# dropbox/lepton

Measured on AMD Instinct MI355X. Metric: encode+decode MB/s (JPEG bytes/sec), bit-exact round trip, higher is better.
Workload: dtype int16/u8 (integer coder, no floating point)

## Files before the change

### lepton_amd/csrc/lep_enc5.h

```cpp
#pragma once
#include "lep_v3.h"
#include "lep_enc5_plan.h"
#ifdef LEP5_DEBUG
#include <cstdio>
#endif

namespace lep5 {
using namespace lep3;

constexpr int kRows = 64, kClasses = 10;
constexpr int kPRows = 63 + 14;
constexpr int kStreams = 2 * kRows * kClasses;
WDEV int stream_id(int ci, int row, int k) { return (ci * kRows + row) * kClasses + k; }
constexpr int kCoefSlice = 12 * 11 + 10 + 1;
constexpr int kSignSlice = 48, kNzSlice = 6 * 32, kEdgeNzSlice = 8 * 12, kDcSlice = 17 * 11 + 10 + 1;
constexpr uint32_t kThreshWords = 2u * 256 * 8 * 128;

WDEV uint32_t coef_entry(uint32_t vlow, int nres, int len, int bsr, int k, int u) {
    return vlow | ((uint32_t)nres << 10) | ((uint32_t)len << 14) | ((uint32_t)bsr << 18) | ((uint32_t)k << 23) | ((uint32_t)u << 27);
}
WDEV int coef_units(int len, int nres) { return ((len < 11 ? len + 1 : 11) + nres + 3) >> 2; }
WDEV uint32_t thresh_entry(uint32_t tbits, int n, int pcls, int lt, int u) {
    return tbits | ((uint32_t)n << 10) | ((uint32_t)pcls << 14) | ((uint32_t)lt << 23) | ((uint32_t)u << 27);
}
// ... 241 lines not shown
}
WDEV void fold_edgenz_wave(const SegPlan5* plans, uint8_t* arena, int seg0, int nseg, int ci, int vertical, int eob, FoldShared* sh) {
    fold_init(sh, kEdgeNzSlice);
    LANES(l) {
        const int seg = seg0 + l;
        if (seg < nseg) {
            const SegPlan5& P = plans[seg];
            const uint32_t* ctab = reinterpret_cast<const uint32_t*>(arena + P.arena_off + P.cls_base);
            const int c = (vertical ? kClsEv : kClsEh) + ci * 8 + eob;
            const uint32_t n = P.status ? 0u : ctab[kNumCls + c];
            uint32_t* rec = reinterpret_cast<uint32_t*>(arena + P.arena_off + P.ens_base[vertical]) + (size_t)(n ? ctab[c] : 0u);
            FoldLane fl{sh->slice + fold_col(l)};
            U4 nxt = n ? ld4(rec) : U4{0, 0, 0, 0};
            for (uint32_t i = 0; i < n; i += 4) {
                U4 g = nxt;
                if (i + 4 < n) nxt = ld4(rec + i + 4);
                uint32_t w[4] = {g.x, g.y, g.z, g.w};
#pragma unroll
                for (int q = 0; q < 4; ++q) {
                    const int nzq = (int)w[q] & 7, ne = (int)(w[q] >> 3) & 7;
                    uint32_t probs = 0;
                    int so_far = 0;
#pragma unroll
                    for (int b = 2; b >= 0; --b) {
                        const uint32_t bit = (uint32_t)(ne >> b) & 1u;
                        probs |= fl.code(nzq * 12 + b * 4 + so_far, bit) << (8 * (2 - b));
                        so_far = (so_far << 1) | (int)bit;
                    }
                    w[q] = probs;
                }
                st4(rec + i, U4{w[0], w[1], w[2], w[3]});
            }
        }
    }
}
WDEV void fold_dc_wave(const SegPlan5* plans, uint8_t* arena, int seg0, int nseg, int a, FoldShared* sh) {
    fold_init(sh, kDcSlice);
    LANES(l) {
        const int seg = seg0 + l;
        if (seg < nseg) {
            const SegPlan5& P = plans[seg];
            const uint32_t* ctab = reinterpret_cast<const uint32_t*>(arena + P.arena_off + P.cls_base);
            const uint32_t n = P.status ? 0u : ctab[kNumCls + kClsDc + a];
            uint32_t* rec = reinterpret_cast<uint32_t*>(arena + P.arena_off + P.dcs_base) + 6 * (size_t)(n ? ctab[kClsDc + a] : 0u);
            FoldLane fl{sh->slice + fold_col(l)};
            uint32_t nxt = n ? rec[0] : 0u;
            for (uint32_t i = 0; i < n; ++i) {
                const uint32_t e0 = nxt;
                if (i + 1 < n) nxt = rec[6 * (i + 1)];
                const int nu = coef_units((int)(e0 >> 14) & 15, (int)(e0 >> 10) & 15);
                for (int u = 0; u < nu; ++u) rec[6 * i + u] = fold_coef_unit(fl, e0 | ((uint32_t)u << 27), 17 * 11);
            }
        }
    }
}

struct BoolEnc5 {
    uint64_t low;
    uint32_t q24;
    int count;
    uint64_t stage;
    int nst;
    uint8_t* out;
    uint32_t pos, cap;
    uint32_t floor_;
    uint32_t carry_out;
    WDEV void init(uint8_t* o, uint32_t c) { out = o; cap = c; pos = 0; low = 0; q24 = 254u << 24; count = -24; stage = 0; nst = 0; floor_ = 0; carry_out = 0; }
    WDEV void bin(uint32_t bit, uint32_t prob) {
#if LEP_ON_GPU
        const uint32_t s = __umulhi(q24, prob);
#else
        const uint32_t s = (uint32_t)(((uint64_t)q24 * prob) >> 32);
#endif
        const uint32_t q = q24 >> 24;
        const uint32_t n = bit ? q - s : s + 1;
        const int f = __builtin_clz(n);
        q24 = (n << f) - (1u << 24);
        low += bit ? s + 1 : 0u;
        low <<= f - 24;
        count += f - 24;
    }
    WDEV void ripple() {
        uint32_t x = pos;
        while (x > floor_ && (x > cap || out[x - 1] == 0xffu)) { if (x <= cap) out[x - 1] = 0; --x; }
        if (x > floor_) out[x - 1] = (uint8_t)(out[x - 1] + 1);
        else if (floor_) ++carry_out;
    }
    WDEV void flush() {
        const int nb = count >= 0 ? (count >> 3) + 1 : 0;
        count -= 8 * nb;
        const int keep = 32 + count;
        const uint64_t o = low >> keep;
        low &= (1ull << keep) - 1;
        stage = (stage << (8 * nb)) + o;
        nst += nb;
        if ((stage >> (8 * nst)) & 1u) { stage &= (1ull << (8 * nst)) - 1; ripple(); }
        if (nst >= 4) {
            const uint32_t v = (uint32_t)(stage >> (8 * (nst - 4)));
            if (pos + 4 <= cap) { const uint32_t be = __builtin_bswap32(v); __builtin_memcpy(out + pos, &be, 4); }
            else for (int i = 0; i < 4; ++i) if (pos + (uint32_t)i < cap) out[pos + i] = (uint8_t)(v >> (24 - 8 * i));
            pos += 4; nst -= 4;
            stage &= (1ull << (8 * nst)) - 1;
        }
    }
    WDEV uint32_t finish(bool* overflow) {
        flush();
// ... 1172 lines not shown
```

### lepton_amd/csrc/lep_gpu.hip

```cpp
#include <hip/hip_runtime.h>

#include <algorithm>
#include <cstdio>
#include <cstdlib>
#include <cstring>
#include <mutex>
#include <string>
#include <vector>

#include "../../include/lepton_mi355x.h"
#include "lep_buffers.h"

#define LEP_DEV __device__ __forceinline__
#include "lep_core.h"
#include "lep_enc3.h"
#include "lep_dec4.h"
#include "lep_enc5.h"
#include "lep_enc5_plan.h"
#include "lep_huff.h"
#include "lep_huffdec.h"
#include "lep_huffdec_simt.h"
#include "lep_huff_simt.h"
#include "lep_huffprog.h"
#include "lep_huffprog_simt.h"
// ... 180 lines not shown
        if (PHASE == 2) __builtin_amdgcn_s_setprio(3);
        if (PHASE == 0) lep5::wchunk_range_lane(plans[seg], bins, recs + (size_t)seg * K + k, k, K);
        else lep5::wchunk_code_lane(plans[seg], bins, segs[seg], streams, recs + (size_t)seg * K + k, k, K);
    } else {
        if (id >= nseg) return;
        if (PHASE == 1) { status[segs[id].slot] = 0; nbins_out[segs[id].slot] = plans[id].nbins; lep5::wchunk_link_lane(plans[id], bins, recs + (size_t)id * K, K); }
        else lep5::wchunk_stitch_lane(plans[id], segs[id], streams, stream_len, status, recs + (size_t)id * K, K);
    }
}
template <int PHASE>
__global__ __launch_bounds__(64) void lep_enc5_wchunk_part_kernel(const lep5::SegPlan5* __restrict__ plans, const uint16_t* __restrict__ bins, const SegDev* __restrict__ segs,
                                                              int nseg, int nparts, int c, int part, lep5::WChunk5* recs, uint8_t* streams, const uint8_t* __restrict__ arena,
                                                              int32_t* status, uint32_t* nbins_out) {
    __builtin_amdgcn_s_setprio(3);
    const int id = (int)(blockIdx.x * 64 + threadIdx.x);
    const int seg = PHASE == 1 ? id : id / c, s = PHASE == 1 ? 0 : id - seg * c;
    if (seg >= nseg) return;
    const lep5::SegPlan5& P = plans[seg];
    const lep5::Ckpt5* ck = reinterpret_cast<const lep5::Ckpt5*>(arena + P.arena_off + P.ckpt_base);
    lep5::WChunk5* r = recs + (size_t)seg * (size_t)(nparts * c);
    if (PHASE == 0) lep5::wchunk_range_cut(P, bins, r + part * c + s, lep5::part_chunk_cut(P, ck, part, s, nparts, c));
    else if (PHASE == 2) lep5::wchunk_code_cut(P, bins, segs[seg], streams, r + part * c + s, lep5::part_chunk_cut(P, ck, part, s, nparts, c));
    else {
        if (part == 0) status[segs[seg].slot] = 0;
        if (part + 1 == nparts) nbins_out[segs[seg].slot] = P.nbins;
        lep5::wchunk_link_cuts(P, bins, r, part * c, (part + 1) * c, [&](int j) { return lep5::part_chunk_cut(P, ck, j / c, j % c, nparts, c); });
    }
}
__global__ void lep_enc5_plan_kernel(const uint32_t* __restrict__ counts, lep5::SegPlan5* plans, int nseg) {
    const int s = (int)(blockIdx.x * blockDim.x + threadIdx.x);
    if (s < nseg) lep5::plan_segment(counts + (size_t)s * lep5::kCountWords, plans + s);
}
__global__ __launch_bounds__(64) void lep_enc5_offsets_kernel(lep5::SegPlan5* plans, int nseg, uint64_t* totals) {
    uint64_t a = 0, b = 0;
    for (int s0 = 0; s0 < nseg; s0 += 64) {
        const int s = s0 + (int)threadIdx.x;
        const uint32_t ab = s < nseg ? plans[s].arena_bytes : 0u, bc = s < nseg ? plans[s].bins_cap : 0u;
        int oa, ob;
        const int va = (int)(ab >> 8), vb = (int)(bc >> 7);
        const int ta = lepwave::wave_excl_scan(&va, &oa), tb = lepwave::wave_excl_scan(&vb, &ob);
        if (s < nseg) { plans[s].arena_off = a + ((uint64_t)(uint32_t)oa << 8); plans[s].bins_off = b + ((uint64_t)(uint32_t)ob << 7); }
        a += (uint64_t)(uint32_t)ta << 8; b += (uint64_t)(uint32_t)tb << 7;
    }
    if (threadIdx.x == 0) { totals[0] = a; totals[1] = b; }
}
__global__ void lep_enc5_fill_kernel(uint4* p, size_t n16, uint32_t v) {
    const uint4 x = make_uint4(v, v, v, v);
    for (size_t i = blockIdx.x * (size_t)blockDim.x + threadIdx.x; i < n16; i += (size_t)gridDim.x * blockDim.x) p[i] = x;
}
__global__ __launch_bounds__(64) void lep_enc5_bucket_kernel(const lep5::SegPlan5* __restrict__ plans, uint8_t* arena) {
    __shared__ lep5::BucketShared sh;
    lep5::bucket_wave(plans + blockIdx.x, arena, &sh);
}
struct Fold5CoefShared { uint16_t slice[lep5::kCoefSlice * 64]; };
__global__ __launch_bounds__(64) void lep_enc5_fold_coef_kernel(const lep5::SegPlan5* __restrict__ plans, uint8_t* arena, int nseg, int groups) {
    __shared__ Fold5CoefShared shc;
    const int grp = (int)blockIdx.x % groups, job = (int)blockIdx.x / groups;
    const int ci = job / 630, row = (job % 630) / 10, k = job % 10;
    const int sid = lep5::stream_id(ci, row, k), seg = grp * 64 + (int)threadIdx.x;
    const bool work = seg < nseg && !plans[seg].status && plans[seg].cnt[sid] != 0;
    if (!__ballot(work)) return;
    lep5::fold_coef_wave(plans, arena, grp * 64, nseg, sid, reinterpret_cast<lep5::FoldShared*>(&shc));
}
struct Fold5SmallShared { uint16_t slice[lep5::kEdgeNzSlice * 64]; };
__global__ __launch_bounds__(64) void lep_enc5_fold_small_kernel(const lep5::SegPlan5* __restrict__ plans, uint8_t* arena, uint32_t* thresh_models, int nseg, int groups, int job0) {
    __shared__ Fold5SmallShared shs;
    lep5::FoldShared* sh = reinterpret_cast<lep5::FoldShared*>(&shs);
    const int grp = (int)blockIdx.x % groups;
    int job = (int)blockIdx.x / groups + job0;
    const int seg0 = grp * 64;
    if (job < 2) { lep5::fold_sign_wave(plans, arena, seg0, nseg, job, sh); return; }
    job -= 2;
    if (job < 12) { const int ci = job / 6, lt = 2 + job % 6; lep5::fold_thresh_wave(plans, arena, thresh_models, seg0, nseg, lep5::stream_id(ci, 63, lt), ci, sh); return; }
    job -= 12;
    lep5::fold_edgenz_wave(plans, arena, seg0, nseg, job / 16, (job / 8) & 1, job & 7, sh);
}
constexpr int kFold5SmallJobs = 2 + 12 + 32;
__global__ __launch_bounds__(64) void lep_enc5_fold_big_kernel(const lep5::SegPlan5* __restrict__ plans, uint8_t* arena, int nseg, int groups, int job0) {
    __shared__ lep5::FoldShared sh;
    const int grp = (int)blockIdx.x % groups;
    int job = (int)blockIdx.x / groups + job0;
    const int seg0 = grp * 64;
    if (job < 12) { lep5::fold_dc_wave(plans, arena, seg0, nseg, job, &sh); return; }
    job -= 12;
    lep5::fold_nz_wave(plans, arena, seg0, nseg, job / 10, job % 10, &sh);
}
constexpr int kFold5BigJobs = 12 + 20;
__global__ __launch_bounds__(64) void lep_enc5_write_kernel(const lep5::SegPlan5* __restrict__ plans, const uint16_t* __restrict__ bins, const SegDev* __restrict__ segs,
                                                          int nseg, uint8_t* streams, uint32_t* stream_len, int32_t* status, uint32_t* nbins_out, uint8_t* arena,
                                                          int part, int nparts) {
    __builtin_amdgcn_s_setprio(3);
    const int seg0 = (int)blockIdx.x * 64, seg = seg0 + (int)threadIdx.x;
    if (seg < nseg) {
        if (part == 0) status[segs[seg].slot] = 0;
        if (part + 1 == nparts) nbins_out[segs[seg].slot] = plans[seg].nbins;
    }
    lep5::write_wave(plans, bins, segs, seg0, nseg, streams, stream_len, status, arena, part, nparts);
}

__global__ __launch_bounds__(64, 8) void lep_huffman_encode_kernel(const lephuff::HuffImage* __restrict__ images,
                                                                   const lephuff::HuffSegment* __restrict__ segs, uint8_t* out,
                                                                   uint32_t* out_len, lephuff::HuffEnd* ends) {
    __shared__ lephuff::HuffShared sh;
    const int s = blockIdx.x;
    const lephuff::HuffSegment seg = segs[s];
    if (seg.pad & lephuff::kHuffSegSimt) return;
    if (seg.pad & lephuff::kHuffSegRefuse) {
        if (threadIdx.x == 0) {
            out_len[s] = 0;
            if (ends) { lephuff::HuffEnd e; memset(&e, 0, sizeof e); e.pad = lephuff::kHuffEndRefused; ends[s] = e; }
        }
        return;
    }
    lephuff::HuffWave w;
    const uint32_t n = w.run(images + seg.image, seg, &sh, out);
    if (threadIdx.x == 0) out_len[s] = n;
    if (ends) w.export_end(ends + s);
}
__global__ __launch_bounds__(256) void lep_zero_kernel(uint4* p, size_t n16) {
    for (size_t i = (size_t)blockIdx.x * blockDim.x + threadIdx.x; i < n16; i += (size_t)gridDim.x * blockDim.x) p[i] = uint4{0u, 0u, 0u, 0u};
}
__global__ __launch_bounds__(leppack::kScanLanes) void lep_pack_offsets_kernel(const uint32_t* __restrict__ len, int n, uint64_t* __restrict__ dst_off) {
    leppack::offsets([len](int i) { return len[i]; }, n, dst_off);
}
__global__ __launch_bounds__(64) void lep_pack_copy_kernel(const uint8_t* __restrict__ src, const uint64_t* __restrict__ src_off, const uint32_t* __restrict__ len,
                                                           int n, uint8_t* __restrict__ dst, uint64_t dst_cap, const uint64_t* __restrict__ dst_off) {
    if (dst_off[n] > dst_cap) return;
    const int i = (int)blockIdx.x;
    leppack::copy_run(src + src_off[i], dst + dst_off[i], len[i], threadIdx.x & 63u);
}
__global__ __launch_bounds__(64 * lepsamples::kWavesPerGroup) void lep_samples_kernel(const lepsamples::PlaneRec* __restrict__ recs, const uint32_t* __restrict__ first, int nplanes) {
    __shared__ uint32_t tiles[lepsamples::kWavesPerGroup][lepsamples::kTileWords];
    const int wave = __builtin_amdgcn_readfirstlane((int)(threadIdx.x >> 6));
    const uint32_t unit = blockIdx.x * (uint32_t)lepsamples::kWavesPerGroup + (uint32_t)wave;
    if (unit >= first[nplanes]) return;
    lepsamples::wave_samples(recs, first, nplanes, unit, tiles[wave]);
}
__global__ __launch_bounds__(64 * lepsamples::kWavesPerGroup) void lep_samples_dc_kernel(const lepsamples::PlaneRec* __restrict__ recs, const uint32_t* __restrict__ first, int nplanes) {
    const int wave = __builtin_amdgcn_readfirstlane((int)(threadIdx.x >> 6));
    const uint32_t unit = blockIdx.x * (uint32_t)lepsamples::kWavesPerGroup + (uint32_t)wave;
// ... 128 lines not shown
    lephuff::prog_rst_reduce(scans + blockIdx.x, plans + blockIdx.x, outs, rows);
}
__global__ __launch_bounds__(64, 4) void lep_huffman_progressive_pipelined_kernel(const lephuff::ProgDecScan* __restrict__ scans, lephuff::HuffDecRow* rows,
                                                                                 const lephuff::ProgDeps* __restrict__ deps, uint32_t* progress, uint32_t* ticket) {
    __shared__ lephuff::HuffDecShared sh;
    uint32_t t = 0;
    if (threadIdx.x == 0) t = atomicAdd(ticket, 1u);
    const int k = __builtin_amdgcn_readfirstlane((int)t);
    lephuff::ProgDecWave w;
    w.run_scan<true>(scans + k, &sh, rows, deps + k, progress, k);
}

__global__ __launch_bounds__(64, 8) void lep_huffman_decode_kernel(const lephuff::HuffDecImage* __restrict__ images, lephuff::HuffDecRow* rows) {
    __shared__ lephuff::HuffDecShared sh;
    __builtin_amdgcn_s_setprio(3);
    lephuff::HuffDecWave w;
    w.run(images + blockIdx.x, &sh, rows);
}

__global__ __launch_bounds__(64) void lep_huffman_simt_settle_kernel(const lephuff::HuffDecImage* __restrict__ images, lephuff::SimtImage* si, const lephuff::SimtWave* waves,
                                                                     const lephuff::SimtSub* in, lephuff::SimtSub* out, int settle, lephuff::SimtSlots* slots) {
    __shared__ lephuff::SimtShared sh;
    extern __shared__ __attribute__((aligned(16))) unsigned char simt_columns[];
    const lephuff::SimtWave w = waves[blockIdx.x];
    lephuff::simt_guess_or_settle(images + w.image, &sh, si + w.image, in + si[w.image].first, out + si[w.image].first, w.first_sub, settle, slots,
                                  reinterpret_cast<lephuff::SimtColumns*>(simt_columns));
}
__global__ __launch_bounds__(64) void lep_huffman_simt_place_kernel(const lephuff::HuffDecImage* __restrict__ images, lephuff::SimtImage* si, const lephuff::SimtSub* sub,
                                                                    lephuff::SimtPlace* place, int passes, lephuff::HuffDecRow* rows, const lephuff::SimtSlots* slots) {
    const int i = (int)blockIdx.x;
    lephuff::simt_place(images + i, si + i, sub + si[i].first, place + si[i].first, passes, rows, slots);
}
__global__ __launch_bounds__(64) void lep_huffman_simt_write_kernel(const lephuff::HuffDecImage* __restrict__ images, lephuff::SimtImage* si, const lephuff::SimtWave* waves,
                                                                    const lephuff::SimtSub* sub, const lephuff::SimtPlace* place, lephuff::HuffDecRow* rows) {
    __shared__ lephuff::SimtShared sh;
    __shared__ lephuff::SimtTile tile;
    const lephuff::SimtWave w = waves[blockIdx.x];
    lephuff::simt_write(images + w.image, &sh, &tile, si + w.image, sub + si[w.image].first, place + si[w.image].first, rows, w.first_sub);
}
__global__ void lep_huffman_simt_finish_kernel(const lephuff::HuffDecImage* __restrict__ images, int nimg, lephuff::HuffDecRow* rows, const lephuff::SimtImage* si) {
    const int i = (int)(blockIdx.x * blockDim.x + threadIdx.x);
    if (i < nimg) lephuff::simt_finish(images + i, si + i, rows);
}

}

struct lep_gpu {
    int device = 0;
    hipStream_t stream = nullptr;
    hipEvent_t ev0 = nullptr, ev1 = nullptr;
    bool timed = false;
    bool released = false;
    lep5::Enc5Options opt;
    hipStream_t stream2 = nullptr, stream3 = nullptr;
    hipEvent_t ev_fork = nullptr, ev_join = nullptr, ev_join3 = nullptr;
    int huffprog_pipeline = 1;
    int huffprog_split = 0;
    int huffprogdec_rst = 1;
    uint32_t huffprogdec_rst_floor = lephuff::kRstPieceFloor;
    int huffprogdec_win = 1;
    int huffprog_simt = 1;
    int huffprog_simt_rst = 1;
    uint32_t huffprog_forms[4] = {0, 0, 0, 0};
    int cut_progressive = 0;
    int stream_pack = 1;
    int huffenc_simt = 1;
    int simt_sub_bits = 0;
    int huffprog_pipeline_max = 16384;
    hipEvent_t ev_part[8] = {nullptr, nullptr, nullptr, nullptr, nullptr, nullptr, nullptr, nullptr};
    int wchunks_parts = 0, wchunks_per_part = 0;
    std::vector<uint32_t> wchunks_slots;
    hipEvent_t ev_stage[8] = {nullptr, nullptr, nullptr, nullptr, nullptr, nullptr, nullptr, nullptr};
    int nstage = 0;
    int dec_company = 0;
    int dec_waves = 0;
    std::string err;
    const char* last_kernel = "";
    char simt_name[112] = "";
    struct Vmm {
        bool on = false;
        size_t chunk = (size_t)512 << 20;
        hipMemAllocationProp prop;
        hipMemAccessDesc access;
        std::vector<hipMemGenericAllocationHandle_t> pool;
        size_t mapped_total = 0, creates = 0, releases = 0;
    } vmm;
    enum Ws {
        W_ENC5_ENTRIES,
        W_ENC5_BINLIST,
        W_MODELS, W_MODELS_1,
        W_NS, W_NS_1,
        W_TRIMMED,
        W_META = W_TRIMMED, W_META_1,
        W_ROWS, W_ROWS_1,
        W_ENC5_PLANS,
        W_ENC5_WCHUNKS,
        W_BLOCKS, W_STREAMS, W_LENS,
        W_HUFF, W_HUFF_1,
        W_HUFFENC, W_HUFFENC_1,
        W_HUFFPROG, W_HUFFPROG_1,
        W_HUFFPROGSIMT, W_HUFFPROGSIMT_1,
        W_HUFFSEQ, W_HUFFSEQ_1,
        W_HUFFPROGDEC,
        W_HUFFPROGRST,
        W_HUFFDEC,
        W_HUFFPAR,
        W_PACK, W_PACK_1,
        W_SAMPLES, W_SAMPLES_1,
// ... 120 lines not shown
    }
    if (b.mapped > old) HIPCHK(g, hipMemSetAccess(b.va + old, b.mapped - old, &V.access, 1));
    w.set(b.va, b.mapped);
    return 0;
}
static int ensure(lep_gpu* g, Workspace& w, size_t need, bool may_release = true) {
    if (w.cap >= need) return 0;
    if (g->vmm.on && (need >= ((size_t)32 << 20) || w.v.va)) {
        if (!w.v.va) HIPCHK(g, w.release());
        return vmm_ensure(g, w, need, may_release);
    }
    hipError_t e = w.ensure(need, need / 8);
    if (e != hipSuccess && may_release) {
        (void)hipGetLastError();
        release_idle_caches(g);
        e = w.ensure(need);
    }
    if (e != hipSuccess) { g->err = std::string("hipMalloc: ") + hipGetErrorString(e); return LEP_GPU_ERROR; }
    return 0;
}

#include "lep_derive.h"


template <class Ready>
static int launch_enc5_writer(const lep5::Enc5WriterPlan& W, const lep5::SegPlan5* plans, const uint16_t* binlist, const SegDev* segs, int nseg, lep5::WChunk5* recs,
                              uint8_t* arena, uint8_t* streams, uint32_t* stream_len, int32_t* status, uint32_t* bins, hipStream_t wst, Ready&& ready) {
#define LEP_WCHUNK(PHASE, GRID) hipLaunchKernelGGL((lep_enc5_wchunk_kernel<PHASE>), dim3(GRID), dim3(64), 0, wst, plans, binlist, segs, nseg, W.records, recs, streams, stream_len, status, bins)
#define LEP_WPART(PHASE, GRID) hipLaunchKernelGGL((lep_enc5_wchunk_part_kernel<PHASE>), dim3(GRID), dim3(64), 0, wst, plans, binlist, segs, nseg, \
                                                  W.gather_parts, W.chunks, part, recs, streams, (const uint8_t*)arena, status, bins)
    for (int part = 0; part < W.gather_parts; ++part) {
        if (int rc = ready(part)) return rc;
        if (W.form == LEP_DEBUG_WRITE_LANE)
            hipLaunchKernelGGL(lep_enc5_write_kernel, dim3(W.groups), dim3(64), 0, wst, plans, binlist, segs, nseg, streams, stream_len, status, bins, arena, part, W.gather_parts);
        if (W.form == LEP_DEBUG_WRITE_PART_CHUNKS) { LEP_WPART(0, W.lane_groups); LEP_WPART(1, W.groups); LEP_WPART(2, W.lane_groups); }
    }
    if (int rc = ready(W.gather_parts)) return rc;
    if (W.form == LEP_DEBUG_WRITE_STITCHED) { LEP_WCHUNK(0, W.lane_groups); LEP_WCHUNK(1, W.groups); LEP_WCHUNK(2, W.lane_groups); }
    if (W.form != LEP_DEBUG_WRITE_LANE) LEP_WCHUNK(3, W.groups);
#undef LEP_WPART
#undef LEP_WCHUNK
    return 0;
}

constexpr int kEnc5NoMemory = -1000;
static int launch_enc5(lep_gpu* g, const ImageDev* d_img, const SegDev* d_seg, const uint64_t* d_nsoff, int nseg, uint8_t* d_streams,
                       uint32_t* d_stream_len, int32_t* d_status, hipStream_t st) {
    Workspace &models = g->ws[lep_gpu::W_MODELS + g->cur], &ns = g->ws[lep_gpu::W_NS + g->cur];
    Workspace &ws_plans = g->ws[lep_gpu::W_ENC5_PLANS], &ws_entries = g->ws[lep_gpu::W_ENC5_ENTRIES], &ws_binlist = g->ws[lep_gpu::W_ENC5_BINLIST], &wchunks = g->ws[lep_gpu::W_ENC5_WCHUNKS];
    if (!g->stream2) {
        HIPCHK(g, hipEventCreateWithFlags(&g->ev_enc5_done, hipEventDisableTiming));
        for (auto& e : g->ev_part) HIPCHK(g, hipEventCreateWithFlags(&e, hipEventDisableTiming));
        HIPCHK(g, hipStreamCreateWithFlags(&g->stream2, hipStreamNonBlocking));
        HIPCHK(g, hipStreamCreateWithFlags(&g->stream3, hipStreamNonBlocking));
        HIPCHK(g, hipEventCreateWithFlags(&g->ev_fork, hipEventDisableTiming));
        HIPCHK(g, hipEventCreateWithFlags(&g->ev_join, hipEventDisableTiming));
        HIPCHK(g, hipEventCreateWithFlags(&g->ev_join3, hipEventDisableTiming));
        for (auto& e : g->ev_stage) HIPCHK(g, hipEventCreate(&e));
    }
    lepbuf::Layout L;
    L.add<lep5::SegPlan5>((size_t)nseg);
    const size_t o_counts = L.add<uint32_t>((size_t)nseg * lep5::kCountWords), o_tot = L.add<uint64_t>(2);
    HIPCHK(g, hipStreamWaitEvent(st, g->ev_enc5_done, 0));
    if (int rc = ensure(g, ws_plans, L.padded())) return rc;
    lep5::SegPlan5* plans = ws_plans.at<lep5::SegPlan5>(0);
    uint32_t* counts = ws_plans.at<uint32_t>(o_counts);
    uint64_t* d_tot = ws_plans.at<uint64_t>(o_tot);
    const int groups = (nseg + 63) / 64;
    g->nstage = 0;
    HIPCHK(g, hipEventRecord(g->ev_stage[0], st));
    const bool two = g->opt.enc5_waves == 2;
    lep5::Enc5WriterPlan W = lep5::enc5_writer_plan(nseg, g->opt);
    int nparts = lep5::enc5_lane_plan(nseg, g->opt).gather_parts;
    auto walk =[&](int mode, uint8_t* entries, uint16_t* binlist, int part = 0) {
        size_t lds = lep5::walk_lds_bytes(mode);
        if (mode == lep5::kGather && g->opt.enc5_gather_wgs > 0) lds = std::max(lds, (size_t)(160 * 1024 / g->opt.enc5_gather_wgs) & ~(size_t)255);
#define LEP_WALK(MODE, NW) hipLaunchKernelGGL((lep_enc5_walk_kernel<MODE, NW>), dim3(nseg), dim3(64 * NW), lds, st, d_img, d_seg, (NSum*)ns.p, d_nsoff, plans, entries, binlist, counts, part, nparts)
        if (mode == lep5::kCount) { if (two) LEP_WALK(lep5::kCount, 2); else LEP_WALK(lep5::kCount, 1); }
        else if (mode == lep5::kEmit) { if (two) LEP_WALK(lep5::kEmit, 2); else LEP_WALK(lep5::kEmit, 1); }
        else { if (two) LEP_WALK(lep5::kGather, 2); else LEP_WALK(lep5::kGather, 1); }
#undef LEP_WALK
    };
    walk(lep5::kCount, nullptr, nullptr);
    hipLaunchKernelGGL(lep_enc5_plan_kernel, dim3(groups), dim3(64), 0, st, (const uint32_t*)counts, plans, nseg);
    hipLaunchKernelGGL(lep_enc5_offsets_kernel, dim3(1), dim3(64), 0, st, plans, nseg, d_tot);
    hipLaunchKernelGGL(lep_enc5_fill_kernel, dim3(4096), dim3(256), 0, st, (uint4*)models.p, (size_t)nseg * lep5::kThreshWords / 4, kBranchInit);
    uint64_t tot[2] = {0, 0};
    HIPCHK(g, hipMemcpyAsync(tot, d_tot, sizeof tot, hipMemcpyDeviceToHost, st));
    HIPCHK(g, hipStreamSynchronize(st));
    if ((size_t)tot[0] + (size_t)tot[1] * 2 > g->opt.enc5_scratch_max || ensure(g, ws_entries, (size_t)tot[0] + 256, false) || ensure(g, ws_binlist, (size_t)tot[1] * 2 + 256, false)) {
        (void)hipGetLastError();
        g->err.clear();
        static bool told = false;
        if (!told) { told = true; fprintf(stderr, "lepton-mi355x: no room for the split-phase encoder's scratch (%.1f GB for %d segments): single-kernel encoder\n", ((double)tot[0] + 2.0 * (double)tot[1]) / 1e9, nseg); }
        return kEnc5NoMemory;
    }
    if (W.records && ensure(g, wchunks, (size_t)nseg * W.records * sizeof(lep5::WChunk5) + 256, false)) { (void)hipGetLastError(); g->err.clear(); W = lep5::enc5_lane_plan(nseg, g->opt); }
    nparts = W.gather_parts;
    {
        HIPCHK(g, hipEventRecord(g->ev_stage[1], st));
        walk(lep5::kEmit, (uint8_t*)ws_entries.p, nullptr);
        HIPCHK(g, hipEventRecord(g->ev_stage[2], st));
        hipLaunchKernelGGL(lep_enc5_bucket_kernel, dim3(nseg), dim3(64), 0, st, (const lep5::SegPlan5*)plans, (uint8_t*)ws_entries.p);
        HIPCHK(g, hipEventRecord(g->ev_fork, st));
        HIPCHK(g, hipStreamWaitEvent(g->stream2, g->ev_fork, 0));
        HIPCHK(g, hipStreamWaitEvent(g->stream3, g->ev_fork, 0));
        if (g->opt.enc5_fold_apart) {
            const int small0[4] = {0, 2, 14, 46}, big0[3] = {0, 12, 32};
            for (int i = 0; i < 3; ++i)
                hipLaunchKernelGGL(lep_enc5_fold_small_kernel, dim3((unsigned)groups * (small0[i + 1] - small0[i])), dim3(64), 0, st, (const lep5::SegPlan5*)plans, (uint8_t*)ws_entries.p,
                                   (uint32_t*)models.p, nseg, groups, small0[i]);
            for (int i = 0; i < 2; ++i)
                hipLaunchKernelGGL(lep_enc5_fold_big_kernel, dim3((unsigned)groups * (big0[i + 1] - big0[i])), dim3(64), 0, st, (const lep5::SegPlan5*)plans, (uint8_t*)ws_entries.p, nseg, groups, big0[i]);
        } else {
        hipLaunchKernelGGL(lep_enc5_fold_small_kernel, dim3((unsigned)groups * kFold5SmallJobs), dim3(64), 0, g->stream2, (const lep5::SegPlan5*)plans, (uint8_t*)ws_entries.p,
                           (uint32_t*)models.p, nseg, groups, 0);
        hipLaunchKernelGGL(lep_enc5_fold_big_kernel, dim3((unsigned)groups * kFold5BigJobs), dim3(64), 0, g->stream3, (const lep5::SegPlan5*)plans, (uint8_t*)ws_entries.p, nseg, groups, 0);
        }
        hipLaunchKernelGGL(lep_enc5_fold_coef_kernel, dim3((unsigned)groups * 1260u), dim3(64), 0, st, (const lep5::SegPlan5*)plans, (uint8_t*)ws_entries.p, nseg, groups);
        HIPCHK(g, hipEventRecord(g->ev_join, g->stream2));
        HIPCHK(g, hipEventRecord(g->ev_join3, g->stream3));
        HIPCHK(g, hipStreamWaitEvent(st, g->ev_join, 0));
        HIPCHK(g, hipStreamWaitEvent(st, g->ev_join3, 0));
        HIPCHK(g, hipEventRecord(g->ev_stage[3], st));
        const hipStream_t wst = W.form == LEP_DEBUG_WRITE_STITCHED ? st : g->stream2;
        auto gathered = [&](int part) -> int {
            if (part == nparts) { HIPCHK(g, hipEventRecord(g->ev_stage[4], st)); return 0; }
            walk(lep5::kGather, (uint8_t*)ws_entries.p, (uint16_t*)ws_binlist.p, part);
            if (wst != st) { HIPCHK(g, hipEventRecord(g->ev_part[part], st)); HIPCHK(g, hipStreamWaitEvent(wst, g->ev_part[part], 0)); }
            return 0;
        };
        if (int rc = launch_enc5_writer(W, plans, (const uint16_t*)ws_binlist.p, d_seg, nseg, (lep5::WChunk5*)wchunks.p, (uint8_t*)ws_entries.p, d_streams, d_stream_len, d_status,
                                        g->d_bins, wst, gathered)) return rc;
        if (wst != st) { HIPCHK(g, hipEventRecord(g->ev_join, wst)); HIPCHK(g, hipStreamWaitEvent(st, g->ev_join, 0)); }
        HIPCHK(g, hipEventRecord(g->ev_stage[5], st));
        g->nstage = 5;
    }
    HIPCHK(g, hipEventRecord(g->ev_enc5_done, st));
    HIPCHK(g, hipGetLastError());
    g->wchunks_parts = W.report_parts; g->wchunks_per_part = W.chunks; g->last_kernel = W.name;
    return 0;
}

#define LEP_STAGED(T, N) static_assert(sizeof(T) == N, "a staged descriptor changed size: tests/test_stage_block.py WORKSPACES and tests/emu/stage_block_probe.cc ELEM_SIZES name it")
LEP_STAGED(ImageDev, 2208); LEP_STAGED(SegDev, 32); LEP_STAGED(lep_huff_image, 4272); LEP_STAGED(lep_huff_segment, 40); LEP_STAGED(lephuff::SimtEncSeg, 40);
LEP_STAGED(lephuff::SimtEncWave, 8); LEP_STAGED(lepsamples::PlaneRec, 176); LEP_STAGED(leprgb::RgbRec, 112); LEP_STAGED(lep_huffprog_image, 168); LEP_STAGED(lep_huffprog_scan, 4184);
LEP_STAGED(lephuff::ProgSimtScan, 48); LEP_STAGED(lephuff::ProgSimtWave, 8); LEP_STAGED(lephuff::ProgSimtRegion, 24); LEP_STAGED(lep_huffprogdec_scan, 5696);
LEP_STAGED(lephuff::ProgDeps, 16); LEP_STAGED(lephuff::ProgRstScan, 16); LEP_STAGED(lephuff::ProgRstOut, 24); LEP_STAGED(lep_huffdec_image, 5552);
LEP_STAGED(lephuff::SimtImage, 36); LEP_STAGED(lephuff::SimtWave, 8); LEP_STAGED(lephuff::SimtSub, 20); LEP_STAGED(lephuff::SimtPlace, 12); LEP_STAGED(lephuff::SimtSlots, 32);

static int stage(lep_gpu* g, Workspace& ws, const lepbuf::Block& B, hipStream_t st) {
    if (int rc = ensure(g, ws, B.padded())) return rc;
    const size_t n = B.upload_bytes();
    if (!n) return 0;
    lep_gpu::Staging& sl = g->staging[g->staging_next];
    g->staging_next = (g->staging_next + 1) % 16;
    if (sl.used) { HIPCHK(g, hipEventSynchronize(sl.ev)); sl.used = false; }
    if (!sl.ev) HIPCHK(g, hipEventCreateWithFlags(&sl.ev, hipEventDisableTiming));
    if (sl.cap < n) {
        if (sl.host) g->staging_retired.push_back(sl.host);
        sl.host = nullptr; sl.cap = 0;
        const size_t want = std::max<size_t>(n + n / 4 + 4096, (size_t)8 << 20);
        HIPCHK(g, hipHostMalloc(&sl.host, want, hipHostMallocDefault));
        sl.cap = want;
    }
    B.pack((char*)sl.host);
    HIPCHK(g, hipMemcpyAsync(ws.p, sl.host, n, hipMemcpyHostToDevice, st));
    HIPCHK(g, hipEventRecord(sl.ev, st));
    sl.used = true;
    return 0;
}

static int refuse_if_session(lep_gpu* g, const char* what) {
    if (!g->rows[g->cur].open) return 0;
    g->err = std::string(what) + ": arena set " + std::to_string(g->cur) + " belongs to a decode session until lep_gpu_decode_rows_end";
    return LEP_ASSERTION_FAILURE;
// ... 123 lines not shown
__attribute__((constructor)) static void lep_runtime_defaults() { setenv("GPU_MAX_HW_QUEUES", "8", 0); }

extern "C" {

static std::mutex g_live_mu;
static std::vector<lep_gpu*> g_live;
static bool g_exit_hook = false;
static void release_device_side(lep_gpu* g);
static void release_all_at_exit() {
    std::lock_guard<std::mutex> lk(g_live_mu);
    for (lep_gpu* g : g_live) release_device_side(g);
    g_live.clear();
}

int lep_gpu_create(int device, lep_gpu** out) {
    lep_gpu* g = new lep_gpu;
    g->device = device;
    if (const char* e = getenv("LEP_DEC_WAVES")) g->dec_waves = atoi(e) == 4 ? 4 : (atoi(e) == 8 ? 8 : 0);
    lep5::enc5_options_from_env(&g->opt);
    if (const char* e = getenv("LEP_HUFFPROG_PIPELINE")) g->huffprog_pipeline = atoi(e);
    if (const char* e = getenv("LEP_HUFFPROG_PIPELINE_MAX")) g->huffprog_pipeline_max = atoi(e);
    if (const char* e = getenv("LEP_HUFFDEC_SIMT_BITS")) g->simt_sub_bits = std::max(0, atoi(e));
    if (const char* e = getenv("LEP_HUFFENC_SIMT")) g->huffenc_simt = atoi(e) != 0;
    if (const char* e = getenv("LEP_STREAM_PACK")) g->stream_pack = atoi(e) != 0;
    if (const char* e = getenv("LEP_CUT_PROGRESSIVE")) g->cut_progressive = atoi(e) != 0;
    if (const char* e = getenv("LEP_HUFFPROG_SIMT")) g->huffprog_simt = atoi(e) != 0;
    if (const char* e = getenv("LEP_HUFFPROG_SIMT_RST")) g->huffprog_simt_rst = atoi(e) != 0;
    if (const char* e = getenv("LEP_HUFFPROGDEC_WIN")) g->huffprogdec_win = atoi(e) != 0;
    if (const char* e = getenv("LEP_HUFFPROGDEC_RST")) g->huffprogdec_rst = atoi(e) != 0;
    if (const char* e = getenv("LEP_HUFFPROGDEC_RST_FLOOR")) g->huffprogdec_rst_floor = (uint32_t)std::max(1, atoi(e));
    if (const char* e = getenv("LEP_HUFFPROG_SPLIT")) g->huffprog_split = atoi(e) != 0;
    int n = 0;
    if (hipGetDeviceCount(&n) != hipSuccess || n <= device) { delete g; return LEP_GPU_ERROR; }
    if (hipSetDevice(device) != hipSuccess || hipStreamCreate(&g->stream) != hipSuccess ||
        hipEventCreate(&g->ev0) != hipSuccess || hipEventCreate(&g->ev1) != hipSuccess) { delete g; return LEP_GPU_ERROR; }
    vmm_init(g);
    {
        std::lock_guard<std::mutex> lk(g_live_mu);
        g_live.push_back(g);
        if (!g_exit_hook) { g_exit_hook = true; atexit(release_all_at_exit); }
    }
    *out = g;
    return 0;
}

static void release_device_side(lep_gpu* g) {
    if (g->released) return;
    g->released = true;
    (void)hipSetDevice(g->device);
    (void)hipStreamSynchronize(g->stream);
    if (g->ev_enc5_done) (void)hipEventDestroy(g->ev_enc5_done);
    for (auto& e : g->ev_part) if (e) (void)hipEventDestroy(e);
    for (auto& e : g->ev_stage) if (e) (void)hipEventDestroy(e);
    if (g->ev_fork) (void)hipEventDestroy(g->ev_fork);
    if (g->ev_join) (void)hipEventDestroy(g->ev_join);
    if (g->ev_join3) (void)hipEventDestroy(g->ev_join3);
    if (g->stream2) (void)hipStreamDestroy(g->stream2);
    if (g->stream3) (void)hipStreamDestroy(g->stream3);
    for (Workspace& w : g->ws) dev_release(g, w);
    vmm_destroy(g);
    if (g->ev0) (void)hipEventDestroy(g->ev0);
    if (g->ev1) (void)hipEventDestroy(g->ev1);
    if (g->stream) (void)hipStreamDestroy(g->stream);
    for (lep_gpu::Staging& sl : g->staging) { if (sl.host) (void)hipHostFree(sl.host); if (sl.ev) (void)hipEventDestroy(sl.ev); sl = lep_gpu::Staging(); }
    for (void* p : g->staging_retired) (void)hipHostFree(p);
    g->staging_retired.clear();
}

void lep_gpu_destroy(lep_gpu* g) {
    if (!g) return;
    {
        std::lock_guard<std::mutex> lk(g_live_mu);
        for (size_t i = 0; i < g_live.size(); ++i) if (g_live[i] == g) { g_live.erase(g_live.begin() + i); break; }
        release_device_side(g);
    }
    delete g;
}

const char* lep_gpu_last_error(lep_gpu* g) { return g ? g->err.c_str() : "no gpu object"; }

int lep_gpu_encode_device(lep_gpu* g, const lep_image_desc* images, int nimg, const lep_segment* segs, int nseg,
                          uint8_t* d_streams, const uint64_t* stream_offsets, uint32_t* d_stream_len, int32_t* d_status,
                          void* hip_stream) {
    return launch<false>(g, images, nimg, segs, nseg, d_streams, stream_offsets, d_stream_len, d_status,
                         hip_stream ? (hipStream_t)hip_stream : g->stream);
}

int lep_gpu_decode_device(lep_gpu* g, const lep_image_desc* images, int nimg, const lep_segment* segs, int nseg,
                          const uint8_t* d_streams, const uint64_t* stream_offsets, const uint32_t* d_stream_len,
                          int32_t* d_status, void* hip_stream) {
    return launch<true>(g, images, nimg, segs, nseg, const_cast<uint8_t*>(d_streams), stream_offsets,
                        const_cast<uint32_t*>(d_stream_len), d_status, hip_stream ? (hipStream_t)hip_stream : g->stream);
}

int lep_gpu_decode_rows_begin(lep_gpu* g, const lep_image_desc* images, int nimg, const lep_segment* segs, int nseg,
                              const uint8_t* d_streams, const uint64_t* stream_offsets, const uint32_t* d_stream_len, void* hip_stream) {
    if (!g) return LEP_GPU_ERROR;
    if (int rc = refuse_if_session(g, "lep_gpu_decode_rows_begin")) return rc;
    if (nseg <= 0 || nimg <= 0) { g->err = "lep_gpu_decode_rows_begin: nothing to decode"; return LEP_ASSERTION_FAILURE; }
    hipStream_t st = hip_stream ? (hipStream_t)hip_stream : g->stream;
    LaunchFront F;
    if (int rc = launch_front(g, true, images, nimg, segs, nseg, stream_offsets, st, &F)) return rc;
    Workspace& recs = g->ws[lep_gpu::W_ROWS + g->cur];
    lepbuf::Layout L;
    L.add<lep4::Dec4Resume>((size_t)nseg);
    L.add<uint32_t>((size_t)nseg * kRowsLdsWords);
    if (int rc = ensure(g, recs, L.bytes())) return rc;
    HIPCHK(g, hipMemsetAsync(recs.p, 0, L.bytes(), st));
    lep_gpu::RowsSession& R = g->rows[g->cur];
    R.nseg = nseg; R.st = st; R.waves = decoder_waves(g, nseg);
    R.d_img = F.d_img; R.d_seg = F.d_seg; R.d_nsoff = F.d_nsoff; R.d_models = F.d_models; R.d_ns = F.d_ns;
// ... 835 lines not shown
```

Before: 1735.

## Merge three fold kernels into one launch and drop the extra streams

Replaces the separate small, big and coef fold kernels, which ran on three streams with fork/join events, with a single fold kernel that decodes a flat job index into a fold kind and dispatches to it. By default every fold job goes out in one grid on the main stream, removing the cross-stream events and two extra launches. All blocks now reserve the largest shared-memory layout, which can reduce occupancy for the small jobs. It also adds optional compile-time priority boosts for the sign and DC jobs, which are off by default.

```diff
diff --git a/lepton_amd/csrc/lep_enc5.h b/lepton_amd/csrc/lep_enc5.h
--- a/lepton_amd/csrc/lep_enc5.h
+++ b/lepton_amd/csrc/lep_enc5.h
@@ -317,6 +317,37 @@
                 for (int u = 0; u < nu; ++u) rec[6 * i + u] = fold_coef_unit(fl, e0 | ((uint32_t)u << 27), 17 * 11);
             }
         }
+    }
+}
+
+enum FoldKind { kFoldSign = 0, kFoldThresh, kFoldDc, kFoldNz, kFoldEdgeNz, kFoldCoef, kFoldKinds };
+constexpr int kFoldJobs = 2 + 12 + 12 + 20 + 32 + 1260;
+constexpr int fold_kind_job0(int kind) {
+    return kind <= kFoldSign ? 0 : kind == kFoldThresh ? 2 : kind == kFoldDc ? 14 : kind == kFoldNz ? 26 : kind == kFoldEdgeNz ? 46 : kind == kFoldCoef ? 78 : kFoldJobs;
+}
+struct FoldJob { int kind, a, b, c; };
+WDEV FoldJob fold_job(int job) {
+    if (job < 2) return FoldJob{kFoldSign, job, 0, 0};
+    job -= 2;
+    if (job < 12) return FoldJob{kFoldThresh, job / 6, 2 + job % 6, 0};
+    job -= 12;
+    if (job < 12) return FoldJob{kFoldDc, job, 0, 0};
+    job -= 12;
+    if (job < 20) return FoldJob{kFoldNz, job / 10, job % 10, 0};
+    job -= 20;
+    if (job < 32) return FoldJob{kFoldEdgeNz, job / 16, (job / 8) & 1, job & 7};
+    job -= 32;
+    return FoldJob{kFoldCoef, job / 630, (job % 630) / 10, job % 10};
+}
+WDEV void fold_run_job(int job, const SegPlan5* plans, uint8_t* arena, uint32_t* thresh_models, int seg0, int nseg, FoldShared* sh) {
+    const FoldJob j = fold_job(job);
+    switch (j.kind) {
+    case kFoldSign: fold_sign_wave(plans, arena, seg0, nseg, j.a, sh); break;
+    case kFoldThresh: fold_thresh_wave(plans, arena, thresh_models, seg0, nseg, stream_id(j.a, 63, j.b), j.a, sh); break;
+    case kFoldDc: fold_dc_wave(plans, arena, seg0, nseg, j.a, sh); break;
+    case kFoldNz: fold_nz_wave(plans, arena, seg0, nseg, j.a, j.b, sh); break;
+    case kFoldEdgeNz: fold_edgenz_wave(plans, arena, seg0, nseg, j.a, j.b, j.c, sh); break;
+    default: fold_coef_wave(plans, arena, seg0, nseg, stream_id(j.a, j.b, j.c), sh); break;
     }
 }
 
diff --git a/lepton_amd/csrc/lep_gpu.hip b/lepton_amd/csrc/lep_gpu.hip
--- a/lepton_amd/csrc/lep_gpu.hip
+++ b/lepton_amd/csrc/lep_gpu.hip
@@ -256,40 +256,27 @@
     __shared__ lep5::BucketShared sh;
     lep5::bucket_wave(plans + blockIdx.x, arena, &sh);
 }
-struct Fold5CoefShared { uint16_t slice[lep5::kCoefSlice * 64]; };
-__global__ __launch_bounds__(64) void lep_enc5_fold_coef_kernel(const lep5::SegPlan5* __restrict__ plans, uint8_t* arena, int nseg, int groups) {
-    __shared__ Fold5CoefShared shc;
-    const int grp = (int)blockIdx.x % groups, job = (int)blockIdx.x / groups;
-    const int ci = job / 630, row = (job % 630) / 10, k = job % 10;
-    const int sid = lep5::stream_id(ci, row, k), seg = grp * 64 + (int)threadIdx.x;
-    const bool work = seg < nseg && !plans[seg].status && plans[seg].cnt[sid] != 0;
-    if (!__ballot(work)) return;
-    lep5::fold_coef_wave(plans, arena, grp * 64, nseg, sid, reinterpret_cast<lep5::FoldShared*>(&shc));
-}
-struct Fold5SmallShared { uint16_t slice[lep5::kEdgeNzSlice * 64]; };
-__global__ __launch_bounds__(64) void lep_enc5_fold_small_kernel(const lep5::SegPlan5* __restrict__ plans, uint8_t* arena, uint32_t* thresh_models, int nseg, int groups, int job0) {
-    __shared__ Fold5SmallShared shs;
-    lep5::FoldShared* sh = reinterpret_cast<lep5::FoldShared*>(&shs);
-    const int grp = (int)blockIdx.x % groups;
-    int job = (int)blockIdx.x / groups + job0;
+#ifndef LEP_ENC5_FOLD_PRIO_SIGN
+#define LEP_ENC5_FOLD_PRIO_SIGN 0
+#endif
+#ifndef LEP_ENC5_FOLD_PRIO_DC
+#define LEP_ENC5_FOLD_PRIO_DC 0
+#endif
+__global__ __launch_bounds__(64) void lep_enc5_fold_kernel(const lep5::SegPlan5* __restrict__ plans, uint8_t* arena, uint32_t* thresh_models, int nseg, int groups, int job0) {
+    __shared__ lep5::FoldShared sh;
+    const int grp = (int)blockIdx.x % groups, job = (int)blockIdx.x / groups + job0;
     const int seg0 = grp * 64;
-    if (job < 2) { lep5::fold_sign_wave(plans, arena, seg0, nseg, job, sh); return; }
-    job -= 2;
-    if (job < 12) { const int ci = job / 6, lt = 2 + job % 6; lep5::fold_thresh_wave(plans, arena, thresh_models, seg0, nseg, lep5::stream_id(ci, 63, lt), ci, sh); return; }
-    job -= 12;
-    lep5::fold_edgenz_wave(plans, arena, seg0, nseg, job / 16, (job / 8) & 1, job & 7, sh);
-}
-constexpr int kFold5SmallJobs = 2 + 12 + 32;
-__global__ __launch_bounds__(64) void lep_enc5_fold_big_kernel(const lep5::SegPlan5* __restrict__ plans, uint8_t* arena, int nseg, int groups, int job0) {
-    __shared__ lep5::FoldShared sh;
-    const int grp = (int)blockIdx.x % groups;
-    int job = (int)blockIdx.x / groups + job0;
-    const int seg0 = grp * 64;
-    if (job < 12) { lep5::fold_dc_wave(plans, arena, seg0, nseg, job, &sh); return; }
-    job -= 12;
-    lep5::fold_nz_wave(plans, arena, seg0, nseg, job / 10, job % 10, &sh);
-}
-constexpr int kFold5BigJobs = 12 + 20;
+    if (job >= lep5::fold_kind_job0(lep5::kFoldCoef)) {
+        const lep5::FoldJob j = lep5::fold_job(job);
+        const int sid = lep5::stream_id(j.a, j.b, j.c), seg = seg0 + (int)threadIdx.x;
+        const bool work = seg < nseg && !plans[seg].status && plans[seg].cnt[sid] != 0;
+        if (!__ballot(work)) return;
+    }
+    if ((LEP_ENC5_FOLD_PRIO_SIGN && job < lep5::fold_kind_job0(lep5::kFoldSign + 1)) ||
+        (LEP_ENC5_FOLD_PRIO_DC && job >= lep5::fold_kind_job0(lep5::kFoldDc) && job < lep5::fold_kind_job0(lep5::kFoldDc + 1)))
+        __builtin_amdgcn_s_setprio(3);
+    lep5::fold_run_job(job, plans, arena, thresh_models, seg0, nseg, &sh);
+}
 __global__ __launch_bounds__(64) void lep_enc5_write_kernel(const lep5::SegPlan5* __restrict__ plans, const uint16_t* __restrict__ bins, const SegDev* __restrict__ segs,
                                                           int nseg, uint8_t* streams, uint32_t* stream_len, int32_t* status, uint32_t* nbins_out, uint8_t* arena,
                                                           int part, int nparts) {
@@ -524,8 +511,8 @@
     bool timed = false;
     bool released = false;
     lep5::Enc5Options opt;
-    hipStream_t stream2 = nullptr, stream3 = nullptr;
-    hipEvent_t ev_fork = nullptr, ev_join = nullptr, ev_join3 = nullptr;
+    hipStream_t stream2 = nullptr;
+    hipEvent_t ev_join = nullptr;
     int huffprog_pipeline = 1;
     int huffprog_split = 0;
     int huffprogdec_rst = 1;
@@ -752,10 +739,7 @@
         HIPCHK(g, hipEventCreateWithFlags(&g->ev_enc5_done, hipEventDisableTiming));
         for (auto& e : g->ev_part) HIPCHK(g, hipEventCreateWithFlags(&e, hipEventDisableTiming));
         HIPCHK(g, hipStreamCreateWithFlags(&g->stream2, hipStreamNonBlocking));
-        HIPCHK(g, hipStreamCreateWithFlags(&g->stream3, hipStreamNonBlocking));
-        HIPCHK(g, hipEventCreateWithFlags(&g->ev_fork, hipEventDisableTiming));
         HIPCHK(g, hipEventCreateWithFlags(&g->ev_join, hipEventDisableTiming));
-        HIPCHK(g, hipEventCreateWithFlags(&g->ev_join3, hipEventDisableTiming));
         for (auto& e : g->ev_stage) HIPCHK(g, hipEventCreate(&e));
     }
     lepbuf::Layout L;
@@ -802,26 +786,12 @@
         walk(lep5::kEmit, (uint8_t*)ws_entries.p, nullptr);
         HIPCHK(g, hipEventRecord(g->ev_stage[2], st));
         hipLaunchKernelGGL(lep_enc5_bucket_kernel, dim3(nseg), dim3(64), 0, st, (const lep5::SegPlan5*)plans, (uint8_t*)ws_entries.p);
-        HIPCHK(g, hipEventRecord(g->ev_fork, st));
-        HIPCHK(g, hipStreamWaitEvent(g->stream2, g->ev_fork, 0));
-        HIPCHK(g, hipStreamWaitEvent(g->stream3, g->ev_fork, 0));
-        if (g->opt.enc5_fold_apart) {
-            const int small0[4] = {0, 2, 14, 46}, big0[3] = {0, 12, 32};
-            for (int i = 0; i < 3; ++i)
-                hipLaunchKernelGGL(lep_enc5_fold_small_kernel, dim3((unsigned)groups * (small0[i + 1] - small0[i])), dim3(64), 0, st, (const lep5::SegPlan5*)plans, (uint8_t*)ws_entries.p,
-                                   (uint32_t*)models.p, nseg, groups, small0[i]);
-            for (int i = 0; i < 2; ++i)
-                hipLaunchKernelGGL(lep_enc5_fold_big_kernel, dim3((unsigned)groups * (big0[i + 1] - big0[i])), dim3(64), 0, st, (const lep5::SegPlan5*)plans, (uint8_t*)ws_entries.p, nseg, groups, big0[i]);
-        } else {
-        hipLaunchKernelGGL(lep_enc5_fold_small_kernel, dim3((unsigned)groups * kFold5SmallJobs), dim3(64), 0, g->stream2, (const lep5::SegPlan5*)plans, (uint8_t*)ws_entries.p,
-                           (uint32_t*)models.p, nseg, groups, 0);
-        hipLaunchKernelGGL(lep_enc5_fold_big_kernel, dim3((unsigned)groups * kFold5BigJobs), dim3(64), 0, g->stream3, (const lep5::SegPlan5*)plans, (uint8_t*)ws_entries.p, nseg, groups, 0);
+        for (int kind = 0; kind < lep5::kFoldKinds; ++kind) {
+            const int j0 = g->opt.enc5_fold_apart ? lep5::fold_kind_job0(kind) : 0, j1 = g->opt.enc5_fold_apart ? lep5::fold_kind_job0(kind + 1) : lep5::kFoldJobs;
+            hipLaunchKernelGGL(lep_enc5_fold_kernel, dim3((unsigned)groups * (unsigned)(j1 - j0)), dim3(64), 0, st, (const lep5::SegPlan5*)plans, (uint8_t*)ws_entries.p,
+                               (uint32_t*)models.p, nseg, groups, j0);
+            if (!g->opt.enc5_fold_apart) break;
         }
-        hipLaunchKernelGGL(lep_enc5_fold_coef_kernel, dim3((unsigned)groups * 1260u), dim3(64), 0, st, (const lep5::SegPlan5*)plans, (uint8_t*)ws_entries.p, nseg, groups);
-        HIPCHK(g, hipEventRecord(g->ev_join, g->stream2));
-        HIPCHK(g, hipEventRecord(g->ev_join3, g->stream3));
-        HIPCHK(g, hipStreamWaitEvent(st, g->ev_join, 0));
-        HIPCHK(g, hipStreamWaitEvent(st, g->ev_join3, 0));
         HIPCHK(g, hipEventRecord(g->ev_stage[3], st));
         const hipStream_t wst = W.form == LEP_DEBUG_WRITE_STITCHED ? st : g->stream2;
         auto gathered = [&](int part) -> int {
@@ -1051,11 +1021,8 @@
     if (g->ev_enc5_done) (void)hipEventDestroy(g->ev_enc5_done);
     for (auto& e : g->ev_part) if (e) (void)hipEventDestroy(e);
     for (auto& e : g->ev_stage) if (e) (void)hipEventDestroy(e);
-    if (g->ev_fork) (void)hipEventDestroy(g->ev_fork);
     if (g->ev_join) (void)hipEventDestroy(g->ev_join);
-    if (g->ev_join3) (void)hipEventDestroy(g->ev_join3);
     if (g->stream2) (void)hipStreamDestroy(g->stream2);
-    if (g->stream3) (void)hipStreamDestroy(g->stream3);
     for (Workspace& w : g->ws) dev_release(g, w);
     vmm_destroy(g);
     if (g->ev0) (void)hipEventDestroy(g->ev0);
```

Result: no change. 1749 (median of 6 runs) (+0.8%).
